# jiwoon-ahn/irn

Measured on AMD Instinct MI355X. Metric: images/sec for CAM+random-walk label gen, VOC12 512^2 (random-walk label generation stage), higher is better.
Workload: dtype f32

## Files before the change

### irn_amd/csrc/affinity.hip

```cpp
#include "path_unroll.hpp"

namespace irn {

namespace {

__device__ __forceinline__ float pow_beta(float a, float beta, int beta_int) {
    double b = (double)a;
    if (beta_int > 0) {
        double r = 1.0;
        int e = beta_int;
        while (e) {
            if (e & 1) r *= b;
            b *= b;
            e >>= 1;
        }
        return (float)r;
    }
    return (float)pow(b, (double)beta);
}

template <bool POW>
__global__ __launch_bounds__(256) void affinity_kernel(const AffJob *__restrict__ jobs,
                                                       const int *__restrict__ dir_start8,
                                                       const int *__restrict__ cell_off8, int n_dirs,
// ... 24 lines not shown
    const bool valid = sy < J.sh && sx < J.sw;
    const int base = ly * LW + lx + halo;
    float *out = J.out + (long)sy * J.sw + sx;

    const float *tb = tile + base;
    for (int d = 0; d < n_dirs; ++d) {
        const int k0 = dir_start8[d], k1 = dir_start8[d + 1];
        float m0 = -INFINITY, m1 = -INFINITY;
        for (int k = k0; k < k1; k += 8) {
            const int4 oa = *reinterpret_cast<const int4 *>(cell_off8 + k);
            const int4 ob = *reinterpret_cast<const int4 *>(cell_off8 + k + 4);
            const float a0 = tb[oa.x], a1 = tb[oa.y], a2 = tb[oa.z], a3 = tb[oa.w];
            const float b0 = tb[ob.x], b1 = tb[ob.y], b2 = tb[ob.z], b3 = tb[ob.w];
            m0 = max3(max3(m0, a0, a1), a2, a3);
            m1 = max3(max3(m1, b0, b1), b2, b3);
        }
        const float m = max3(m0, m1, m1);
        float a = 1.0f - m;
        if (POW) a = pow_beta(a, beta, beta_int);
        if (valid) out[(long)d * J.plane_stride] = a;
    }
}

template <int R>
__global__ __launch_bounds__(256) void affinity_unrolled_kernel(const AffJob *__restrict__ jobs, int beta_int) {
    constexpr int HALO = R - 1, LW = AFF_TW + 2 * HALO, LH = AFF_TH + HALO, ND = kPaths<R>.n_dirs;
    __shared__ float tile[LH * LW];
    const AffJob J = jobs[blockIdx.y];
    const int tiles_x = (J.sw + AFF_TW - 1) / AFF_TW;
    const int tiles_y = (J.sh + AFF_TH - 1) / AFF_TH;
    if ((int)blockIdx.x >= tiles_x * tiles_y) return;
    const int ty0 = ((int)blockIdx.x / tiles_x) * AFF_TH;
    const int tx0 = ((int)blockIdx.x % tiles_x) * AFF_TW;
    for (int i = threadIdx.x; i < LH * LW; i += 256) {
        const int ly = i / LW, lx = i - ly * LW;
        const int gy = J.oy + ty0 + ly;
        const int gx = J.ox + tx0 + lx - HALO;
        float v = 1.0f;
        if (gy < J.gh && gx >= 0 && gx < J.gw) v = J.edge[(long)gy * J.gw + gx];
        tile[i] = v;
    }
    __syncthreads();
    const int ly = threadIdx.x / AFF_TW, lx = threadIdx.x % AFF_TW;
    const int sy = ty0 + ly, sx = tx0 + lx;
    const bool valid = sy < J.sh && sx < J.sw;
    const float *tb = tile + ly * LW + lx;
    float *out = J.out + (long)sy * J.sw + sx;
    static_for<ND>([&](auto id) __attribute__((always_inline)) {
        constexpr int d = decltype(id)::value;
        double b = (double)(1.0f - path_max<R, d>(tb)), r = 1.0;
        for (int e = beta_int; e; e >>= 1) {
            if (e & 1) r *= b;
            b *= b;
        }
        if (valid) *out = (float)r;
        out += J.plane_stride;
    });
}

__global__ __launch_bounds__(256) void affinity_backward_kernel(const AffJob *__restrict__ jobs,
                                                                const float *const *__restrict__ grad_aff,
                                                                float *const *__restrict__ grad_edge,
                                                                const int *__restrict__ dir_start,
                                                                const int *__restrict__ cell_dy,
                                                                const int *__restrict__ cell_dx, int n_dirs, int radius) {
    extern __shared__ float tile[];
    const AffJob J = jobs[blockIdx.y];
    const int tiles_x = (J.sw + AFF_TW - 1) / AFF_TW;
    const int tiles_y = (J.sh + AFF_TH - 1) / AFF_TH;
    if ((int)blockIdx.x >= tiles_x * tiles_y) return;
    const int halo = radius - 1;
    const int LW = AFF_TW + 2 * halo;
    const int LH = AFF_TH + halo;
    float *gtile = tile + LH * LW;
    const int ty0 = ((int)blockIdx.x / tiles_x) * AFF_TH;
    const int tx0 = ((int)blockIdx.x % tiles_x) * AFF_TW;
    for (int i = threadIdx.x; i < LH * LW; i += 256) {
        const int ly = i / LW, lx = i - ly * LW;
        const int gy = J.oy + ty0 + ly;
// ... 19 lines not shown
                const float v = tile[base + off];
                if (v > m) {
                    m = v;
                    arg = off;
                }
            }
            atomicAdd(&gtile[base + arg], -ga[(long)d * J.plane_stride]);
        }
    }
    __syncthreads();
    float *ge = grad_edge[blockIdx.y];
    for (int i = threadIdx.x; i < LH * LW; i += 256) {
        const float g = gtile[i];
        if (g == 0.f) continue;
        const int py = i / LW, px = i - py * LW;
        const int gy = J.oy + ty0 + py;
        const int gx = J.ox + tx0 + px - halo;
        if (gy < J.gh && gx >= 0 && gx < J.gw) unsafeAtomicAdd(ge + (long)gy * J.gw + gx, g);
    }
}

}

int launch_affinity(const AffJob *jobs_dev, int n_jobs, int max_sh, int max_sw, const DeviceTable &tab,
                    bool with_pow, float beta, hipStream_t stream) {
    const int tiles = cdiv(max_sh, AFF_TH) * cdiv(max_sw, AFF_TW);
    const int halo = tab.radius - 1;
    const size_t lds = sizeof(float) * (AFF_TH + halo) * (AFF_TW + 2 * halo);
    dim3 grid(tiles, n_jobs);
    int beta_int = 0;
    if (with_pow && beta == (float)(int)beta && beta >= 1.0f && beta <= 64.0f) beta_int = (int)beta;
    if (with_pow && beta_int > 0 && tab.order == 1 && tab.radius == 10)
        hipLaunchKernelGGL(affinity_unrolled_kernel<10>, grid, dim3(256), 0, stream, jobs_dev, beta_int);
    else if (with_pow && beta_int > 0 && tab.order == 1 && tab.radius == 5)
        hipLaunchKernelGGL(affinity_unrolled_kernel<5>, grid, dim3(256), 0, stream, jobs_dev, beta_int);
    else if (with_pow)
        hipLaunchKernelGGL(affinity_kernel<true>, grid, dim3(256), lds, stream, jobs_dev, tab.dir_start8,
                           tab.cell_off8, tab.n_dirs, tab.radius, beta, beta_int);
    else
        hipLaunchKernelGGL(affinity_kernel<false>, grid, dim3(256), lds, stream, jobs_dev, tab.dir_start8,
                           tab.cell_off8, tab.n_dirs, tab.radius, beta, beta_int);
    IRN_LAUNCH_CHECK("affinity_kernel");
    return IRN_OK;
}

}

using namespace irn;

extern "C" int irn_version(void) { return 100; }

extern "C" const char *irn_last_error(void) { return last_error_slot().c_str(); }

extern "C" int irn_path_count(int radius, int *n_dirs, int *n_cells) {
    if (radius < 2 || radius > IRN_MAX_RADIUS || !n_dirs || !n_cells)
        return fail(IRN_ERR_ARG, "irn_path_count: radius must be in [2,%d]", IRN_MAX_RADIUS);
    PathTable t = build_path_table(radius, 0);
    *n_dirs = t.n_dirs();
// ... 160 lines not shown
```

### irn_amd/csrc/kernels.hpp

```cpp
#pragma once
#include "common.hpp"

namespace irn {

struct DeviceTable {
    int radius = 0, order = 0, n_dirs = 0, n_cells = 0;
    int *dir_dy = nullptr, *dir_dx = nullptr;
    int *dir_start = nullptr;
    int *cell_dy = nullptr, *cell_dx = nullptr;
    int *cell_off8 = nullptr;
    int *dir_start8 = nullptr;
    int *plane_tab = nullptr;
    PathTable host;
};

int get_device_table(int radius, int order, const DeviceTable **out);

int scratch_upload(const void *host, size_t bytes, void **dev_out, hipStream_t stream);
int scratch_release(hipStream_t stream);

constexpr int kAffTileH = 8, kAffTileW = 32;

struct AffJob {
    const float *edge;
    float *out;
    int gh, gw;
    int oy, ox;
    int sh, sw;
    long plane_stride;
};

int launch_affinity(const AffJob *jobs_dev, int n_jobs, int max_sh, int max_sw, const DeviceTable &tab,
                    bool with_pow, float beta, hipStream_t stream);

}
```

### irn_amd/csrc/label.hip

```cpp
#include "kernels.hpp"

#pragma clang fp contract(off)

namespace irn {

struct LabelJob {
    const float *rw;
    const int64_t *keys;
    uint8_t *labels;
    int32_t *argmax;
    float *rw_up;
    unsigned *max_slot;
    int c, h, w, oh, ow;
};

namespace {

__device__ __forceinline__ unsigned enc_ordered(float f) {
    const unsigned b = __float_as_uint(f);
    return (b & 0x80000000u) ? ~b : (b | 0x80000000u);
}
__device__ __forceinline__ float dec_ordered(unsigned u) {
    return __uint_as_float((u & 0x80000000u) ? (u & 0x7fffffffu) : ~u);
}
// ... 7 lines not shown
    float src = ((float)dst + 0.5f) * 0.25f;
    src = src - 0.5f;
    src = src < 0.f ? 0.f : src;
    Taps t;
    t.i0 = min((int)src, n_in - 1);
    t.i1 = min(t.i0 + 1, n_in - 1);
    t.l1 = src - (float)t.i0;
    t.l0 = 1.0f - t.l1;
    return t;
}

__device__ __forceinline__ float bilerp(const float *__restrict__ plane, int w, const Taps &ty, const Taps &tx) {
    const float v00 = plane[ty.i0 * w + tx.i0], v01 = plane[ty.i0 * w + tx.i1];
    const float v10 = plane[ty.i1 * w + tx.i0], v11 = plane[ty.i1 * w + tx.i1];
    const float p01 = v01 * tx.l1, p11 = v11 * tx.l1;
    const float top = __builtin_fmaf(v00, tx.l0, p01);
    const float bot = __builtin_fmaf(v10, tx.l0, p11);
    const float pb = ty.l1 * bot;
    return __builtin_fmaf(ty.l0, top, pb);
}

__device__ __forceinline__ int cell_lo(int k) { return k == 0 ? 0 : 4 * k + 2; }

template <int PASS>
__global__ __launch_bounds__(256) void upsample_max_kernel(const LabelJob *__restrict__ jobs) {
    const LabelJob J = jobs[blockIdx.y];
    const unsigned plane_px = (unsigned)(J.h * J.w), cells = (unsigned)J.c * plane_px;
    const float lower = PASS == 2 ? dec_ordered(*J.max_slot) : 0.f;
    float m = -INFINITY;
    for (unsigned i = blockIdx.x * 256 + threadIdx.x; i < cells; i += gridDim.x * 256) {
        const int c = (int)(i / plane_px);
        const int r = (int)(i - (unsigned)c * plane_px);
        const int k = (int)((unsigned)r / (unsigned)J.w), l = r - k * J.w;
        const int y0 = cell_lo(k), x0 = cell_lo(l);
        if (y0 >= J.oh || x0 >= J.ow) continue;
        const float *plane = J.rw + (long)c * J.h * J.w;
        if (PASS == 1) {
            m = fmaxf(m, bilerp(plane, J.w, taps_x4(y0, J.h), taps_x4(x0, J.w)));
        } else {
            const int k1 = min(k + 1, J.h - 1), l1 = min(l + 1, J.w - 1);
            const float u = fmaxf(fmaxf(plane[k * J.w + l], plane[k * J.w + l1]), fmaxf(plane[k1 * J.w + l], plane[k1 * J.w + l1]));
            if (u + fabsf(u) * 1e-6f + 1e-37f < lower) continue;
            const int y1 = min(k == J.h - 1 ? 4 * J.h - 1 : 4 * k + 5, J.oh - 1);
            const int x1 = min(l == J.w - 1 ? 4 * J.w - 1 : 4 * l + 5, J.ow - 1);
            for (int oy = y0; oy <= y1; ++oy) {
                const Taps ty = taps_x4(oy, J.h);
                for (int ox = x0; ox <= x1; ++ox) m = fmaxf(m, bilerp(plane, J.w, ty, taps_x4(ox, J.w)));
            }
        }
    }
    for (int s = 32; s > 0; s >>= 1) m = fmaxf(m, __shfl_xor(m, s));
    __shared__ float wmax[4];
    if ((threadIdx.x & 63) == 0) wmax[threadIdx.x >> 6] = m;
    __syncthreads();
    if (threadIdx.x == 0) {
        m = fmaxf(fmaxf(wmax[0], wmax[1]), fmaxf(wmax[2], wmax[3]));
        if (m > -INFINITY) atomicMax(J.max_slot, enc_ordered(m));
    }
}

__device__ __forceinline__ float bilerp_vals(float v00, float v01, float v10, float v11, const Taps &ty, const Taps &tx) {
    const float p01 = v01 * tx.l1, p11 = v11 * tx.l1;
    const float top = __builtin_fmaf(v00, tx.l0, p01);
    const float bot = __builtin_fmaf(v10, tx.l0, p11);
    const float pb = ty.l1 * bot;
    return __builtin_fmaf(ty.l0, top, pb);
}

__global__ __launch_bounds__(256) void label_argmax_kernel(const LabelJob *__restrict__ jobs, float bg) {
    const LabelJob J = jobs[blockIdx.y];
    const unsigned gw = (unsigned)(J.ow + 3) >> 2, groups = gw * (unsigned)J.oh;
    const unsigned npx = (unsigned)J.oh * (unsigned)J.ow;
    const float gmax = dec_ordered(*J.max_slot);
    for (unsigned g = blockIdx.x * 256 + threadIdx.x; g < groups; g += gridDim.x * 256) {
        const int oy = (int)(g / gw), ox = (int)(g - (unsigned)oy * gw) * 4;
        const int nq = min(4, J.ow - ox);
        const Taps ty = taps_x4(oy, J.h);
        Taps tx[4];
#pragma unroll
        for (int q = 0; q < 4; ++q) tx[q] = taps_x4(min(ox + q, J.ow - 1), J.w);
        float best[4] = {bg, bg, bg, bg};
// ... 122 lines not shown
            out_h[i] > 4 * h[i] || out_w[i] > 4 * w[i])
            return fail(IRN_ERR_ARG, "irn_label_epilogue: image %d: bad sizes (c=%d %dx%d -> %dx%d)", i, c[i], h[i],
                        w[i], out_h[i], out_w[i]);
        J.rw = rw_dev[i];
        J.keys = keys_dev ? keys_dev[i] : nullptr;
        J.labels = labels_dev ? labels_dev[i] : nullptr;
        J.argmax = argmax_dev ? argmax_dev[i] : nullptr;
        J.rw_up = rw_up_dev ? rw_up_dev[i] : nullptr;
        if (J.labels && !J.keys)
            return fail(IRN_ERR_ARG, "irn_label_epilogue: image %d: labels requested without keys", i);
        J.max_slot = (unsigned *)scratch_dev + i;
        J.c = c[i]; J.h = h[i]; J.w = w[i]; J.oh = out_h[i]; J.ow = out_w[i];
        max_px = std::max(max_px, (long)out_h[i] * out_w[i]);
        max_cells = std::max(max_cells, (long)c[i] * h[i] * w[i]);
    }
    LabelJob *jobs_dev = nullptr;
    int rc = scratch_upload(jobs.data(), sizeof(LabelJob) * n_images, (void **)&jobs_dev, stream);
    if (rc) return rc;
    IRN_HIP_TRY(hipMemsetAsync(scratch_dev, 0, sizeof(unsigned) * n_images, stream));
    if (max_px >= (1L << 31) || max_cells >= (1L << 31)) return fail(IRN_ERR_ARG, "irn_label_epilogue: image too large (32-bit pixel indices)");
    const long per_image = std::max<long>(1, 4096 / n_images);
    const int bx = (int)std::min<long>((max_px / 4 + 255) / 256 + 1, 512);
    const int bc = (int)std::min<long>((max_cells + 255) / 256, per_image);
    hipLaunchKernelGGL(upsample_max_kernel<1>, dim3(bc, n_images), dim3(256), 0, stream, jobs_dev);
    IRN_LAUNCH_CHECK("upsample_max_kernel<1>");
    hipLaunchKernelGGL(upsample_max_kernel<2>, dim3(bc, n_images), dim3(256), 0, stream, jobs_dev);
    IRN_LAUNCH_CHECK("upsample_max_kernel<2>");
    hipLaunchKernelGGL(label_argmax_kernel, dim3(bx, n_images), dim3(256), 0, stream, jobs_dev, bg_thres);
    IRN_LAUNCH_CHECK("label_argmax_kernel");
    return scratch_release(stream);
}

extern "C" int irn_cam_merge(int n_scales, const float *const *src_dev, const int32_t *hs, const int32_t *ws, int n_classes,
                             const int64_t *keys_dev, int n_keys, int out_h, int out_w, float *cam_dev,
                             float *high_res_dev, void *scratch_dev, void *stream_) {
    hipStream_t stream = (hipStream_t)stream_;
    if (n_scales < 1 || n_scales > kMaxScales || !src_dev || !hs || !ws || n_classes < 1 || !keys_dev || n_keys < 1 ||
        out_h < 1 || out_w < 1 || !cam_dev || !high_res_dev || !scratch_dev)
        return fail(IRN_ERR_ARG, "irn_cam_merge: bad argument (1..%d scales, >= 1 key)", kMaxScales);
    MergeArgs A;
    for (int s = 0; s < n_scales; ++s) {
        if (!src_dev[s] || hs[s] < 1 || ws[s] < 1) return fail(IRN_ERR_ARG, "irn_cam_merge: scale %d: bad input", s);
        A.src[s] = src_dev[s];
        A.hs[s] = hs[s];
        A.ws[s] = ws[s];
    }
    A.n_scales = n_scales;
    A.n_cls = n_classes;
    A.k = n_keys;
    A.keys = keys_dev;
// ... 18 lines not shown
```

### irn_amd/csrc/path_unroll.hpp

```cpp
#pragma once
#include <utility>

#include "kernels.hpp"

namespace irn {

constexpr int AFF_TH = kAffTileH;
constexpr int AFF_TW = kAffTileW;

__device__ __forceinline__ float max3(float a, float b, float c) {
    float r;
    asm("v_max3_f32 %0, %1, %2, %3" : "=v"(r) : "v"(a), "v"(b), "v"(c));
    return r;
}

template <int R>
struct Paths {
    static constexpr int kMaxDirs = 2 * R * R, kMaxCells = 32 * R * R;
    int n_dirs = 0, n_cells = 0;
    signed char dy[kMaxDirs] = {}, dx[kMaxDirs] = {};
    short start[kMaxDirs + 1] = {};
    signed char cy[kMaxCells] = {}, cx[kMaxCells] = {};
    constexpr void add(int y, int x) {
        dy[n_dirs] = (signed char)y;
        dx[n_dirs] = (signed char)x;
        const int lsq = y * y + x * x;
        const int x_lo = x < 0 ? x : 0, x_hi = x < 0 ? 0 : x;
        for (int py = 0; py <= y; ++py)
            for (int px = x_lo; px <= x_hi; ++px) {
                const int cross = y * px - x * py;
                if (cross * cross < lsq) {
                    cy[n_cells] = (signed char)py;
                    cx[n_cells] = (signed char)px;
                    ++n_cells;
                }
            }
        start[++n_dirs] = (short)n_cells;
    }
    constexpr Paths() {
        for (int x = 1; x < R; ++x) add(0, x);
        for (int y = 1; y < R; ++y)
            for (int x = -R + 1; x < R; ++x)
                if (x * x + y * y < R * R) add(y, x);
    }
};
template <int R>
inline constexpr Paths<R> kPaths{};

template <int... Is, typename F>
__device__ __forceinline__ void static_for_impl(std::integer_sequence<int, Is...>, F &&f) {
    (f(std::integral_constant<int, Is>{}), ...);
}
template <int N, typename F>
__device__ __forceinline__ void static_for(F &&f) {
    static_for_impl(std::make_integer_sequence<int, N>{}, f);
}

template <int R, int D>
__device__ __forceinline__ float path_max(const float *tb) {
    constexpr int LW = AFF_TW + 2 * (R - 1), HALO = R - 1;
    constexpr int k0 = kPaths<R>.start[D], n = kPaths<R>.start[D + 1] - k0;
    constexpr auto off = [](int k) constexpr { return kPaths<R>.cy[k] * LW + kPaths<R>.cx[k] + HALO; };
    float m = tb[off(k0)];
    static_for<(n - 1) / 2>([&](auto ik) __attribute__((always_inline)) {
        constexpr int k = k0 + 1 + 2 * decltype(ik)::value;
        m = max3(m, tb[off(k)], tb[off(k + 1)]);
    });
    if constexpr ((n - 1) % 2 == 1) {
        const float v = tb[off(k0 + n - 1)];
        m = max3(m, v, v);
    }
    return m;
}

}
```

### irn_amd/csrc/walk.hip

```cpp
#include <algorithm>
#include <cmath>
#include <mutex>

#include "walk_ctx.hpp"

namespace irn {


namespace {


__global__ __launch_bounds__(256) void zero_pad_kernel(const WalkImg *__restrict__ imgs, int n_dirs) {
    const WalkImg I = imgs[blockIdx.y];
    const int d = blockIdx.x;
    if (d >= n_dirs) return;
    float *plane = I.wts + (long)d * I.plane_stride;
    for (int i = threadIdx.x; i < I.front_pad; i += 256) plane[-1 - i] = 0.f;
    const long n = (long)I.h * I.w;
    const long end = I.plane_stride - I.front_pad;
    for (long i = n + threadIdx.x; i < end; i += 256) plane[i] = 0.f;
}

__global__ __launch_bounds__(256) void degree_kernel(const WalkImg *__restrict__ imgs,
                                                     const int *__restrict__ dir_dy,
                                                     const int *__restrict__ dir_dx, int n_dirs) {
    const WalkImg I = imgs[blockIdx.y];
    const long n = (long)I.h * I.w;
    const long p = (long)blockIdx.x * 256 + threadIdx.x;
    if (p >= n) return;
    const int y = (int)(p / I.w), x = (int)(p - (long)y * I.w);
    double deg = 1.0;
    for (int d = 0; d < n_dirs; ++d) {
        const int dy = dir_dy[d], dx = dir_dx[d];
        const float *plane = I.wts + (long)d * I.plane_stride;
        deg += (double)plane[p];
        const int yy = y - dy, xx = x - dx;
        if (yy >= 0 && xx >= 0 && xx < I.w) deg += (double)plane[p - ((long)dy * I.w + dx)];
    }
    I.inv_deg[p] = 1.0 / deg;
}

__global__ __launch_bounds__(256) void x0_kernel(const WalkImg *__restrict__ imgs, int to_out, int cheb, float c0) {
    const WalkImg I = imgs[blockIdx.y];
// ... 721 lines not shown
        I.out = out_dev[i];
        I.wts = (float *)(ws + ctx->off_wts[i]) + ctx->front_pad[i];
        I.inv_deg = (double *)(ws + ctx->off_deg[i]);
        I.xa = (float *)(ws + ctx->off_xa[i]);
        I.xb = (float *)(ws + ctx->off_xb[i]);
        I.xc = (float *)(ws + ctx->off_xc[i]);
        I.h = ctx->h[i];
        I.w = ctx->w[i];
        I.C = ctx->c[i];
        I.plane_stride = ctx->plane_stride[i];
        I.front_pad = ctx->front_pad[i];
        I.n_dirs = ctx->tab->n_dirs;
        AffJob &J = jobs[i];
        J.edge = I.edge;
        J.out = I.wts;
        J.gh = I.h; J.gw = I.w; J.oy = 0; J.ox = 0; J.sh = I.h; J.sw = I.w;
        J.plane_stride = I.plane_stride;
    }
    IRN_HIP_TRY(hipMemcpyAsync(ctx->imgs_dev, imgs, sizeof(WalkImg) * n, hipMemcpyHostToDevice, stream));
    IRN_HIP_TRY(hipMemcpyAsync(ctx->jobs_dev, jobs, sizeof(AffJob) * n, hipMemcpyHostToDevice, stream));
    IRN_HIP_TRY(hipEventRecord(ctx->stage_ev[slot], stream));

    const DeviceTable &tab = *ctx->tab;
    hipLaunchKernelGGL(zero_pad_kernel, dim3(tab.n_dirs, n), dim3(256), 0, stream, ctx->imgs_dev, tab.n_dirs);
    IRN_LAUNCH_CHECK("zero_pad_kernel");
    int rc = launch_affinity(ctx->jobs_dev, n, ctx->max_h, ctx->max_w, tab, true, beta, stream);
    if (rc) return rc;
    const bool resident = ctx->variant == 2 && ctx->res_ok && n_sweeps > 0;
    ctx->deg_stale = resident;
    ctx->last_stream = stream;
    ctx->last_n_sweeps = n_sweeps;
    ctx->last_resident = resident;
    ctx->last_valid = true;
    hipEvent_t ev0 = nullptr, ev1 = nullptr;
    if (ctx->timing && resident) {
        rc = timing_events(ctx, &ev0, &ev1);
        if (rc) return rc;
        IRN_HIP_TRY(hipEventRecord(ev0, stream));
    }
    if (resident) {
        rc = resident_run(ctx, n_sweeps, stream);
        if (rc) return rc;
        if (ctx->timing) {
            IRN_HIP_TRY(hipEventRecord(ev1, stream));
            ctx->ev_used += 2;
            ctx->pending_launches += ctx->sched_steps;
        }
    } else {
        rc = streaming_run(ctx, n_sweeps, stream, ctx->timing != 0);
        if (rc) return rc;
    }
    if (!ctx->run_done_ev) IRN_HIP_TRY(hipEventCreateWithFlags(&ctx->run_done_ev, hipEventDisableTiming));
    IRN_HIP_TRY(hipEventRecord(ctx->run_done_ev, stream));
    return IRN_OK;
}

extern "C" int irn_walk_check(irn_walk_ctx *ctx) {
    if (!ctx) return fail(IRN_ERR_ARG, "null ctx");
    if (!ctx->res_err_host) return IRN_OK;
    if (ctx->res_err_host[0] != 0) {
        const unsigned img = ctx->res_err_host[1], t = ctx->res_err_host[2], wg = ctx->res_err_host[3];
        ctx->res_err_host[0] = 0;
        return fail(IRN_ERR_STATE, "resident walk timed out: workgroup %u waiting for state of sweep %u of image %u "
                                   "(a neighbouring tile never published it)", wg, t, img);
// ... 79 lines not shown
```

### irn_amd/csrc/walk_ctx.hpp

```cpp
#pragma once
#include <utility>
#include <vector>

#include "kernels.hpp"

namespace irn {

struct WalkImg {
    const float *edge;
    const float *cam;
    const int *inst;
    float *out;
    float *wts;
    double *inv_deg;
    float *xa, *xb;
    float *xc;
    int h, w, C, k_inst;
    long plane_stride;
    int front_pad, n_dirs;
};

#define IRN_GLOBAL __attribute__((address_space(1)))

template <int R>
__host__ __device__ constexpr bool in_set(int dy, int dx) {
    return dy == 0 ? (dx >= 1 && dx < R) : (dy < R && dx > -R && dx < R && dx * dx + dy * dy < R * R);
}

template <int R>
__host__ __device__ constexpr int plane_of(int dy, int dx) {
    int n = 0;
    for (int y = 0; y < R; ++y)
        for (int x = -R + 1; x < R; ++x) {
            if (y == dy && x == dx) return n;
            if (in_set<R>(y, x)) ++n;
        }
    return -1;
}

template <int... Is, typename F>
__device__ __forceinline__ void static_for_impl(std::integer_sequence<int, Is...>, F &&f) {
    (f(std::integral_constant<int, Is>{}), ...);
}
template <int N, typename F>
__device__ __forceinline__ void static_for(F &&f) {
    static_for_impl(std::make_integer_sequence<int, N>{}, f);
}

}

struct irn_walk_ctx {
    using DeviceTable = irn::DeviceTable;
    using WalkImg = irn::WalkImg;
    using AffJob = irn::AffJob;
    int radius = 0;
    const DeviceTable *tab = nullptr;
    int variant = 1;
    hipStream_t side[3] = {nullptr, nullptr, nullptr};
    hipEvent_t ev_fork = nullptr, ev_join[3] = {nullptr, nullptr, nullptr};
    int n = 0;
    std::vector<int> h, w, c;
    std::vector<size_t> off_wts, off_deg, off_xa, off_xb, off_xc;
    std::vector<long> plane_stride;
    std::vector<int> front_pad;
    size_t ws_bytes = 0;
    int max_h = 0, max_w = 0, max_n = 0;
    bool all_blocked_ok = false;
    WalkImg *imgs_dev = nullptr;
    AffJob *jobs_dev = nullptr;
// ... 31 lines not shown
    bool res_coop_refused = false;
    int res_inject_timeout = 0;
    hipStream_t last_stream = nullptr;
    hipEvent_t run_done_ev = nullptr;
    bool last_valid = false, last_resident = false;
    int last_n_sweeps = 0;
    int fallback_runs = 0;
    int accel = 1;
    int accel_tol_exp = 7;
    int sched_n = -1, sched_accel = -1, sched_tol = -1;
    int sched_steps = 0;
    bool sched_cheb = false;
    float *coef_dev = nullptr;
    std::vector<double> sched_coef;
    std::vector<float> sched_coef_f;
    int coef_cap = 0;
};

namespace irn {
bool resident_supported(const irn_walk_ctx *ctx);
int resident_configure(irn_walk_ctx *ctx);
bool resident_plan_rounds(int radius, int n, const int *h, const int *w, const int *c, int n_wg, int placement,
                          std::vector<int> &jobs, int *n_rounds);
int resident_run(irn_walk_ctx *ctx, int n_sweeps, hipStream_t stream);
int walk_schedule(irn_walk_ctx *ctx, int n_sweeps, hipStream_t stream);
int chebyshev_power_series(int n, double tol, std::vector<double> *coef, bool *cheb);
int streaming_run(irn_walk_ctx *ctx, int n_sweeps, hipStream_t stream, bool timed);
void resident_destroy(irn_walk_ctx *ctx);
}
```

### irn_amd/csrc/walk_resident.hip

```cpp
#include <algorithm>
#include <mutex>

#include "walk_ctx.hpp"

namespace irn {
namespace {

typedef unsigned long long u64;
typedef const double IRN_GLOBAL *gcd_t;
typedef float IRN_GLOBAL *gf_t;
typedef float f4a __attribute__((ext_vector_type(4)));

constexpr int kSlabH = 8, kSlabW = 32;
constexpr int kWaves = 8;
constexpr int kPsLdsBytes = 96 * 1024;

template <int R>
struct RCfg;
template <>
struct RCfg<10> {
    static constexpr int Q = 8, SL_Y = 1, SL_X = 1;
};
template <>
struct RCfg<5> {
    static constexpr int Q = 2, SL_Y = 2, SL_X = 2;
};

template <int R>
struct Disc {
    int n = 0;
    signed char dy[4 * R * R] = {}, dx[4 * R * R] = {};
// ... 189 lines not shown
typedef unsigned u4v __attribute__((ext_vector_type(4)));
constexpr int kSc1 = 16;
__device__ __forceinline__ u2v ld_granule(__amdgpu_buffer_rsrc_t rsrc, int voff, int soff) {
    return __builtin_bit_cast(u2v, __builtin_amdgcn_raw_buffer_load_b64(rsrc, voff, soff, kSc1));
}
template <int AUX = kSc1>
__device__ __forceinline__ void st_granule(__amdgpu_buffer_rsrc_t rsrc, int voff, int soff, unsigned tag, float v) {
    u2v g;
    g.x = __float_as_uint(v);
    g.y = tag;
    __builtin_amdgcn_raw_buffer_store_b64(g, rsrc, voff, soff, AUX);
}

template <int AUX = kSc1>
__device__ __forceinline__ void st_granule2(__amdgpu_buffer_rsrc_t rsrc, int voff, int soff, unsigned tag, float v0, float v1) {
    u4v g;
    g.x = __float_as_uint(v0);
    g.y = tag;
    g.z = __float_as_uint(v1);
    g.w = tag;
    __builtin_amdgcn_raw_buffer_store_b128(g, rsrc, voff, soff, AUX);
}

typedef float f2a __attribute__((ext_vector_type(2)));
__global__ __launch_bounds__(256) void x0_granule_kernel(const WalkImg *__restrict__ imgs, int cheb, float c0) {
    const WalkImg I = imgs[blockIdx.y];
    const long n = (long)I.h * I.w;
    const long p = (long)blockIdx.x * 256 + threadIdx.x;
    if (p >= n) return;
    const float one_minus = 1.0f - I.edge[p];
    const int k = I.inst ? I.k_inst : 1;
    const int id = I.inst ? I.inst[p] : 0;
    u64 *xa = (u64 *)I.xa, *xb = (u64 *)I.xb;
    for (int c = 0; c < I.C; ++c) {
        const int cls = c / k, kk = c - cls * k;
        float v = I.cam[(long)cls * n + p];
        if (I.inst) v = v * (id == kk ? 1.0f : 0.0f);
        xa[(long)c * n + p] = ((u64)1 << 32) | (u64)__float_as_uint(v * one_minus);
        xb[(long)c * n + p] = 0;
        if (cheb) ((f2a *)I.xc)[(long)c * n + p] = f2a{0.f, c0 * (v * one_minus)};
    }
}

__global__ __launch_bounds__(64) void xcc_probe_kernel(unsigned char *__restrict__ out) {
    if (threadIdx.x == 0) out[blockIdx.x] = (unsigned char)((unsigned)__builtin_amdgcn_s_getreg((31 << 11) | 20) & 7u);
}

template <int R, bool PROF>
__global__ __launch_bounds__(512) __attribute__((amdgpu_waves_per_eu(2, 2))) void resident_kernel(
    const WalkImg *__restrict__ imgs, const int4 *__restrict__ jobs, int n_rounds, int t_first, int t_count,
    int t_total, unsigned *err, long long timeout_ticks, long long *prof, int poll_delay, unsigned long long *votes,
    const float *__restrict__ coef, int cheb) {
    using G = Geom<R>;
    constexpr int H = G::H, HP = G::HP, LH = G::LH, LW = G::LW, LWU = G::LWU, RG = G::RG, Q = G::Q, NK = G::NK;
    extern __shared__ __attribute__((aligned(16))) char smem[];
    float *xs = reinterpret_cast<float *>(smem);
    double *part = reinterpret_cast<double *>(smem + G::XS_BYTES);
    double *invd = reinterpret_cast<double *>(smem + G::XS_BYTES + G::PART_BYTES);
    int *abort_flag = reinterpret_cast<int *>(smem + G::XS_BYTES + G::PART_BYTES + G::INVD_BYTES);
    f2a *psl = reinterpret_cast<f2a *>(smem + G::PS_OFF);

    const int tid = threadIdx.x;
    const int lane = tid & 63;
    const int wv = __builtin_amdgcn_readfirstlane(tid >> 6);
// ... 660 lines not shown
    }
    const WalkImg *imgs = ctx->imgs_dev;
    const int4 *jobs = ctx->res_jobs_dev;
    int n_rounds = ctx->res_rounds;
    unsigned *err = ctx->res_err_dev;
    long long *prof = ctx->res_prof_dev;
    int delays = ctx->res_poll_delay | (ctx->res_poll_delay_plain << 16);
    const float *coef = ctx->coef_dev;
    int cheb = ctx->sched_cheb ? 1 : 0;
    if (ctx->res_cooperative && !ctx->res_coop_refused) {
        void *args[] = {&imgs, &jobs, &n_rounds, &t_first, &t_count, &t_total, &err, &ticks, &prof, &delays, &votes, &coef, &cheb};
        const hipError_t e = hipLaunchCooperativeKernel((const void *)resident_kernel<R, PROF>, dim3(ctx->res_nwg), dim3(512),
                                                        args, G::LDS_BYTES, stream);
        if (e == hipSuccess) return IRN_OK;
        (void)hipGetLastError();
        ctx->res_coop_refused = true;
    }
    hipLaunchKernelGGL((resident_kernel<R, PROF>), dim3(ctx->res_nwg), dim3(512), G::LDS_BYTES, stream, imgs, jobs, n_rounds,
                       t_first, t_count, t_total, err, ticks, prof, delays, votes, coef, cheb);
    IRN_LAUNCH_CHECK("resident_kernel");
    return IRN_OK;
}

static int resident_enqueue(irn_walk_ctx *ctx, hipStream_t stream) {
    const int n = ctx->n;
    const int n_sweeps = ctx->sched_steps;
    IRN_HIP_TRY(hipMemsetAsync(ctx->res_err_dev, 0, 4 * sizeof(unsigned), stream));
    hipLaunchKernelGGL(x0_granule_kernel, dim3(cdiv(ctx->max_n, 256), n), dim3(256), 0, stream, ctx->imgs_dev,
                       ctx->sched_cheb ? 1 : 0, ctx->sched_cheb ? (float)ctx->sched_coef[0] : 0.f);
    IRN_LAUNCH_CHECK("x0_granule_kernel");
    const int step = ctx->res_sweeps_per_launch > 0 ? ctx->res_sweeps_per_launch : n_sweeps;
    for (int t = 0; t < n_sweeps; t += step) {
        const int cnt = std::min(step, n_sweeps - t);
        int rc;
        if (ctx->res_prof_dev)
            rc = ctx->radius == 10 ? launch_resident<10, true>(ctx, t, cnt, n_sweeps, stream)
                                   : launch_resident<5, true>(ctx, t, cnt, n_sweeps, stream);
        else
            rc = ctx->radius == 10 ? launch_resident<10, false>(ctx, t, cnt, n_sweeps, stream)
                                   : launch_resident<5, false>(ctx, t, cnt, n_sweeps, stream);
        if (rc) return rc;
    }
    IRN_HIP_TRY(hipMemcpyAsync(ctx->res_err_host, ctx->res_err_dev, 4 * sizeof(unsigned), hipMemcpyDeviceToHost, stream));
    return IRN_OK;
}

static int g_poll_delay[64] = {};

static int resident_probe_poll_delay(irn_walk_ctx *ctx, hipStream_t stream) {
    int dev = 0;
    IRN_HIP_TRY(hipGetDevice(&dev));
    if (dev < 0 || dev >= 64 || ctx->radius != 10 || !ctx->res_poll_auto) return IRN_OK;
    std::lock_guard<std::mutex> lk(g_tune_mu);
    if (g_poll_delay[dev]) {
        ctx->res_poll_delay = g_poll_delay[dev];
        return IRN_OK;
    }
    if (ctx->res_prof_dev || ctx->res_sweeps_per_launch > 0 || ctx->res_inject_timeout || ctx->res_rounds < 4 ||
        ctx->sched_steps < 32)
        return IRN_OK;
    int single = 0;
    for (int i = 0; i < ctx->n; ++i) single += ctx->c[i] == 1 ? 1 : 0;
    if (3 * single < ctx->n) return IRN_OK;
    hipEvent_t e0, e1;
    IRN_HIP_TRY(hipEventCreate(&e0));
    IRN_HIP_TRY(hipEventCreate(&e1));
    constexpr int NC = 4;
    const int cand[NC] = {10, 8, 12, 14};
    float best_ms[NC] = {1e30f, 1e30f, 1e30f, 1e30f};
    int rc = IRN_OK;
    for (int rep = 0; rep < 2 && !rc; ++rep)
        for (int k = 0; k < NC && !rc; ++k) {
            ctx->res_poll_delay = cand[k];
            (void)hipEventRecord(e0, stream);
            rc = resident_enqueue(ctx, stream);
            (void)hipEventRecord(e1, stream);
            if (rc) break;
            if (hipEventSynchronize(e1) != hipSuccess) { rc = fail(IRN_ERR_HIP, "poll-delay probe: synchronisation failed"); break; }
            float ms = 0.f;
            (void)hipEventElapsedTime(&ms, e0, e1);
            if (ctx->res_err_host[0] != 0) ms = 1e30f;
            best_ms[k] = std::min(best_ms[k], ms);
        }
    (void)hipEventDestroy(e0);
    (void)hipEventDestroy(e1);
    int pick = 0;
    for (int k = 1; k < NC; ++k)
        if (best_ms[k] < 0.993f * best_ms[0] && best_ms[k] < best_ms[pick]) pick = k;
    ctx->res_poll_delay = cand[pick];
    ctx->res_poll_probe_ms[0] = best_ms[1];
    ctx->res_poll_probe_ms[1] = best_ms[0];
    ctx->res_poll_probe_ms[2] = best_ms[2];
    ctx->res_poll_probe_ms[3] = best_ms[3];
    if (!rc && best_ms[0] < 1e29f) g_poll_delay[dev] = cand[pick];
    return rc;
}

int resident_run(irn_walk_ctx *ctx, int n_sweeps, hipStream_t stream) {
    {
        const int rc_s = walk_schedule(ctx, n_sweeps, stream);
        if (rc_s) return rc_s;
    }
    {
        const int rc_p = resident_probe_poll_delay(ctx, stream);
        if (rc_p) return rc_p;
    }
    return resident_enqueue(ctx, stream);
}

}
```

Measured before the change: 19280.

## Fuse walk setup into affinity kernel, nest path maxima, single-launch upsample max

The unrolled affinity kernel gains extra blocks that zero the wts plane padding and initialise the x0 granules, which removes the separate zero_pad and x0_granule launches on the resident path. Each direction's path maximum now starts from a parent direction whose cell set is a subset (a compile-time forest), which cuts the LDS reads per pixel considerably. Beta is specialised at compile time for beta=10. The two-pass upsample_max kernels are merged into one kernel that takes its pruning bound from a per-block atomicMax between the passes. That gives a weaker bound than the old global one and may prune less.

```diff
diff --git a/irn_amd/csrc/affinity.hip b/irn_amd/csrc/affinity.hip
--- a/irn_amd/csrc/affinity.hip
+++ b/irn_amd/csrc/affinity.hip
@@ -1,4 +1,5 @@
 #include "path_unroll.hpp"
+#include "walk_setup.hpp"
 
 namespace irn {
 
@@ -70,10 +71,18 @@
     }
 }
 
-template <int R>
-__global__ __launch_bounds__(256) void affinity_unrolled_kernel(const AffJob *__restrict__ jobs, int beta_int) {
+template <int R, int BETA>
+__global__ __launch_bounds__(256) void affinity_unrolled_kernel(const AffJob *__restrict__ jobs, int beta_int, int tiles,
+                                                                AffSetup setup) {
     constexpr int HALO = R - 1, LW = AFF_TW + 2 * HALO, LH = AFF_TH + HALO, ND = kPaths<R>.n_dirs;
     __shared__ float tile[LH * LW];
+    if ((int)blockIdx.x >= tiles) {
+        const WalkImg I = setup.imgs[blockIdx.y];
+        const int b = (int)blockIdx.x - tiles;
+        if (b < ND) zero_pad_plane(I, b);
+        else x0_granules(I, (long)(b - ND) * 256 + threadIdx.x, setup.cheb, setup.c0);
+        return;
+    }
     const AffJob J = jobs[blockIdx.y];
     const int tiles_x = (J.sw + AFF_TW - 1) / AFF_TW;
     const int tiles_y = (J.sh + AFF_TH - 1) / AFF_TH;
@@ -91,18 +100,28 @@
     __syncthreads();
     const int ly = threadIdx.x / AFF_TW, lx = threadIdx.x % AFF_TW;
     const int sy = ty0 + ly, sx = tx0 + lx;
-    const bool valid = sy < J.sh && sx < J.sw;
+    if (sy >= J.sh || sx >= J.sw) return;
     const float *tb = tile + ly * LW + lx;
-    float *out = J.out + (long)sy * J.sw + sx;
-    static_for<ND>([&](auto id) __attribute__((always_inline)) {
-        constexpr int d = decltype(id)::value;
-        double b = (double)(1.0f - path_max<R, d>(tb)), r = 1.0;
-        for (int e = beta_int; e; e >>= 1) {
-            if (e & 1) r *= b;
-            b *= b;
+    typedef __attribute__((address_space(1))) float gfloat;
+    const unsigned pix = (unsigned)sy * (unsigned)J.sw + (unsigned)sx;
+    float chain[kForest<R>.max_depth + 1];
+    static_for<ND>([&](auto ii) __attribute__((always_inline)) {
+        constexpr int i = decltype(ii)::value, d = kForest<R>.order[i];
+        double b = (double)(1.0f - nested_path_max<R, i>(tb, chain)), r = 1.0;
+        if constexpr (BETA > 0) {
+            static_for<32 - __builtin_clz(BETA)>([&](auto ie) __attribute__((always_inline)) {
+                constexpr int e = BETA >> decltype(ie)::value;
+                if constexpr (e & 1) r *= b;
+                if constexpr (e > 1) b *= b;
+            });
+        } else {
+            for (int e = beta_int; e; e >>= 1) {
+                if (e & 1) r *= b;
+                b *= b;
+            }
         }
-        if (valid) *out = (float)r;
-        out += J.plane_stride;
+        ((gfloat *)(J.out + d * J.plane_stride))[pix] = (float)r;
+        if constexpr (i % 4 == 3) __builtin_amdgcn_sched_barrier(0);
     });
 }
 
@@ -168,18 +187,32 @@
 
 }
 
+static int affinity_beta_int(bool with_pow, float beta) {
+    return with_pow && beta == (float)(int)beta && beta >= 1.0f && beta <= 64.0f ? (int)beta : 0;
+}
+
+bool affinity_has_setup_roles(const DeviceTable &tab, float beta) {
+    return affinity_beta_int(true, beta) > 0 && tab.order == 1 && (tab.radius == 5 || tab.radius == 10);
+}
+
 int launch_affinity(const AffJob *jobs_dev, int n_jobs, int max_sh, int max_sw, const DeviceTable &tab,
-                    bool with_pow, float beta, hipStream_t stream) {
+                    bool with_pow, float beta, hipStream_t stream, const AffSetup *setup) {
     const int tiles = cdiv(max_sh, AFF_TH) * cdiv(max_sw, AFF_TW);
     const int halo = tab.radius - 1;
     const size_t lds = sizeof(float) * (AFF_TH + halo) * (AFF_TW + 2 * halo);
-    dim3 grid(tiles, n_jobs);
-    int beta_int = 0;
-    if (with_pow && beta == (float)(int)beta && beta >= 1.0f && beta <= 64.0f) beta_int = (int)beta;
-    if (with_pow && beta_int > 0 && tab.order == 1 && tab.radius == 10)
-        hipLaunchKernelGGL(affinity_unrolled_kernel<10>, grid, dim3(256), 0, stream, jobs_dev, beta_int);
-    else if (with_pow && beta_int > 0 && tab.order == 1 && tab.radius == 5)
-        hipLaunchKernelGGL(affinity_unrolled_kernel<5>, grid, dim3(256), 0, stream, jobs_dev, beta_int);
+    const int beta_int = affinity_beta_int(with_pow, beta);
+    const bool unrolled = beta_int > 0 && tab.order == 1 && (tab.radius == 5 || tab.radius == 10);
+    if (setup && !unrolled) return fail(IRN_ERR_STATE, "launch_affinity: this kernel has no set-up roles");
+    const AffSetup su = setup ? *setup : AffSetup{nullptr, 0, 0, 0.f};
+    dim3 grid(tiles + (setup ? tab.n_dirs + su.x0_blocks : 0), n_jobs);
+    if (unrolled && beta_int == 10 && tab.radius == 10)
+        hipLaunchKernelGGL((affinity_unrolled_kernel<10, 10>), grid, dim3(256), 0, stream, jobs_dev, beta_int, tiles, su);
+    else if (unrolled && beta_int == 10)
+        hipLaunchKernelGGL((affinity_unrolled_kernel<5, 10>), grid, dim3(256), 0, stream, jobs_dev, beta_int, tiles, su);
+    else if (unrolled && tab.radius == 10)
+        hipLaunchKernelGGL((affinity_unrolled_kernel<10, 0>), grid, dim3(256), 0, stream, jobs_dev, beta_int, tiles, su);
+    else if (unrolled)
+        hipLaunchKernelGGL((affinity_unrolled_kernel<5, 0>), grid, dim3(256), 0, stream, jobs_dev, beta_int, tiles, su);
     else if (with_pow)
         hipLaunchKernelGGL(affinity_kernel<true>, grid, dim3(256), lds, stream, jobs_dev, tab.dir_start8,
                            tab.cell_off8, tab.n_dirs, tab.radius, beta, beta_int);
diff --git a/irn_amd/csrc/kernels.hpp b/irn_amd/csrc/kernels.hpp
--- a/irn_amd/csrc/kernels.hpp
+++ b/irn_amd/csrc/kernels.hpp
@@ -30,7 +30,9 @@
     long plane_stride;
 };
 
+struct AffSetup;
+bool affinity_has_setup_roles(const DeviceTable &tab, float beta);
 int launch_affinity(const AffJob *jobs_dev, int n_jobs, int max_sh, int max_sw, const DeviceTable &tab,
-                    bool with_pow, float beta, hipStream_t stream);
+                    bool with_pow, float beta, hipStream_t stream, const AffSetup *setup = nullptr);
 
 }
diff --git a/irn_amd/csrc/label.hip b/irn_amd/csrc/label.hip
--- a/irn_amd/csrc/label.hip
+++ b/irn_amd/csrc/label.hip
@@ -53,11 +53,19 @@
 
 __device__ __forceinline__ int cell_lo(int k) { return k == 0 ? 0 : 4 * k + 2; }
 
-template <int PASS>
+__device__ __forceinline__ float block_max(float m, float *slot) {
+    for (int s = 32; s > 0; s >>= 1) m = fmaxf(m, __shfl_xor(m, s));
+    __syncthreads();
+    if ((threadIdx.x & 63) == 0) slot[threadIdx.x >> 6] = m;
+    __syncthreads();
+    return fmaxf(fmaxf(slot[0], slot[1]), fmaxf(slot[2], slot[3]));
+}
+
 __global__ __launch_bounds__(256) void upsample_max_kernel(const LabelJob *__restrict__ jobs) {
     const LabelJob J = jobs[blockIdx.y];
     const unsigned plane_px = (unsigned)(J.h * J.w), cells = (unsigned)J.c * plane_px;
-    const float lower = PASS == 2 ? dec_ordered(*J.max_slot) : 0.f;
+    __shared__ float wmax[4];
+    __shared__ float lower_s;
     float m = -INFINITY;
     for (unsigned i = blockIdx.x * 256 + threadIdx.x; i < cells; i += gridDim.x * 256) {
         const int c = (int)(i / plane_px);
@@ -65,29 +73,37 @@
         const int k = (int)((unsigned)r / (unsigned)J.w), l = r - k * J.w;
         const int y0 = cell_lo(k), x0 = cell_lo(l);
         if (y0 >= J.oh || x0 >= J.ow) continue;
+        m = fmaxf(m, bilerp(J.rw + (long)c * J.h * J.w, J.w, taps_x4(y0, J.h), taps_x4(x0, J.w)));
+    }
+    m = block_max(m, wmax);
+    if (threadIdx.x == 0) {
+        unsigned seen = 0;
+        if (m > -INFINITY) seen = max(atomicMax(J.max_slot, enc_ordered(m)), enc_ordered(m));
+        lower_s = seen ? dec_ordered(seen) : -INFINITY;
+    }
+    __syncthreads();
+    const float lower = lower_s;
+    if (!(m > -INFINITY)) return;
+    m = -INFINITY;
+    for (unsigned i = blockIdx.x * 256 + threadIdx.x; i < cells; i += gridDim.x * 256) {
+        const int c = (int)(i / plane_px);
+        const int r = (int)(i - (unsigned)c * plane_px);
+        const int k = (int)((unsigned)r / (unsigned)J.w), l = r - k * J.w;
+        const int y0 = cell_lo(k), x0 = cell_lo(l);
+        if (y0 >= J.oh || x0 >= J.ow) continue;
         const float *plane = J.rw + (long)c * J.h * J.w;
-        if (PASS == 1) {
-            m = fmaxf(m, bilerp(plane, J.w, taps_x4(y0, J.h), taps_x4(x0, J.w)));
-        } else {
-            const int k1 = min(k + 1, J.h - 1), l1 = min(l + 1, J.w - 1);
-            const float u = fmaxf(fmaxf(plane[k * J.w + l], plane[k * J.w + l1]), fmaxf(plane[k1 * J.w + l], plane[k1 * J.w + l1]));
-            if (u + fabsf(u) * 1e-6f + 1e-37f < lower) continue;
-            const int y1 = min(k == J.h - 1 ? 4 * J.h - 1 : 4 * k + 5, J.oh - 1);
-            const int x1 = min(l == J.w - 1 ? 4 * J.w - 1 : 4 * l + 5, J.ow - 1);
-            for (int oy = y0; oy <= y1; ++oy) {
-                const Taps ty = taps_x4(oy, J.h);
-                for (int ox = x0; ox <= x1; ++ox) m = fmaxf(m, bilerp(plane, J.w, ty, taps_x4(ox, J.w)));
-            }
-        }
-    }
-    for (int s = 32; s > 0; s >>= 1) m = fmaxf(m, __shfl_xor(m, s));
-    __shared__ float wmax[4];
-    if ((threadIdx.x & 63) == 0) wmax[threadIdx.x >> 6] = m;
-    __syncthreads();
-    if (threadIdx.x == 0) {
-        m = fmaxf(fmaxf(wmax[0], wmax[1]), fmaxf(wmax[2], wmax[3]));
-        if (m > -INFINITY) atomicMax(J.max_slot, enc_ordered(m));
-    }
+        const int k1 = min(k + 1, J.h - 1), l1 = min(l + 1, J.w - 1);
+        const float u = fmaxf(fmaxf(plane[k * J.w + l], plane[k * J.w + l1]), fmaxf(plane[k1 * J.w + l], plane[k1 * J.w + l1]));
+        if (u + fabsf(u) * 1e-6f + 1e-37f < lower) continue;
+        const int y1 = min(k == J.h - 1 ? 4 * J.h - 1 : 4 * k + 5, J.oh - 1);
+        const int x1 = min(l == J.w - 1 ? 4 * J.w - 1 : 4 * l + 5, J.ow - 1);
+        for (int oy = y0; oy <= y1; ++oy) {
+            const Taps ty = taps_x4(oy, J.h);
+            for (int ox = x0; ox <= x1; ++ox) m = fmaxf(m, bilerp(plane, J.w, ty, taps_x4(ox, J.w)));
+        }
+    }
+    m = block_max(m, wmax);
+    if (threadIdx.x == 0 && m > -INFINITY) atomicMax(J.max_slot, enc_ordered(m));
 }
 
 __device__ __forceinline__ float bilerp_vals(float v00, float v01, float v10, float v11, const Taps &ty, const Taps &tx) {
@@ -256,10 +272,8 @@
     const long per_image = std::max<long>(1, 4096 / n_images);
     const int bx = (int)std::min<long>((max_px / 4 + 255) / 256 + 1, 512);
     const int bc = (int)std::min<long>((max_cells + 255) / 256, per_image);
-    hipLaunchKernelGGL(upsample_max_kernel<1>, dim3(bc, n_images), dim3(256), 0, stream, jobs_dev);
-    IRN_LAUNCH_CHECK("upsample_max_kernel<1>");
-    hipLaunchKernelGGL(upsample_max_kernel<2>, dim3(bc, n_images), dim3(256), 0, stream, jobs_dev);
-    IRN_LAUNCH_CHECK("upsample_max_kernel<2>");
+    hipLaunchKernelGGL(upsample_max_kernel, dim3(bc, n_images), dim3(256), 0, stream, jobs_dev);
+    IRN_LAUNCH_CHECK("upsample_max_kernel");
     hipLaunchKernelGGL(label_argmax_kernel, dim3(bx, n_images), dim3(256), 0, stream, jobs_dev, bg_thres);
     IRN_LAUNCH_CHECK("label_argmax_kernel");
     return scratch_release(stream);
diff --git a/irn_amd/csrc/path_unroll.hpp b/irn_amd/csrc/path_unroll.hpp
--- a/irn_amd/csrc/path_unroll.hpp
+++ b/irn_amd/csrc/path_unroll.hpp
@@ -1,7 +1,6 @@
 #pragma once
-#include <utility>
-
 #include "kernels.hpp"
+#include "static_for.hpp"
 
 namespace irn {
 
@@ -47,15 +46,6 @@
 template <int R>
 inline constexpr Paths<R> kPaths{};
 
-template <int... Is, typename F>
-__device__ __forceinline__ void static_for_impl(std::integer_sequence<int, Is...>, F &&f) {
-    (f(std::integral_constant<int, Is>{}), ...);
-}
-template <int N, typename F>
-__device__ __forceinline__ void static_for(F &&f) {
-    static_for_impl(std::make_integer_sequence<int, N>{}, f);
-}
-
 template <int R, int D>
 __device__ __forceinline__ float path_max(const float *tb) {
     constexpr int LW = AFF_TW + 2 * (R - 1), HALO = R - 1;
@@ -73,4 +63,97 @@
     return m;
 }
 
+template <int R>
+struct Forest {
+    static constexpr int kMaxDirs = Paths<R>::kMaxDirs, kMaxCells = Paths<R>::kMaxCells;
+    static constexpr int kRowBits = 2 * R - 1, kWords = (R * kRowBits + 63) / 64;
+    struct Mask {
+        unsigned long long w[kWords] = {};
+        int count = 0;
+        constexpr void set(int y, int x) {
+            const int b = y * kRowBits + x + R - 1;
+            w[b / 64] |= 1ull << (b % 64);
+            ++count;
+        }
+        constexpr bool has(int y, int x) const {
+            const int b = y * kRowBits + x + R - 1;
+            return (w[b / 64] >> (b % 64)) & 1ull;
+        }
+        constexpr bool within(const Mask &o) const {
+            for (int i = 0; i < kWords; ++i)
+                if (w[i] & ~o.w[i]) return false;
+            return true;
+        }
+    };
+    int n_dirs = 0, n_cells = 0, max_depth = 0, operands = 0;
+    short parent[kMaxDirs] = {}, order[kMaxDirs] = {}, depth[kMaxDirs] = {};
+    short start[kMaxDirs + 1] = {};
+    signed char cy[kMaxCells] = {}, cx[kMaxCells] = {};
+    bool exact = true;
+    Mask mask[kMaxDirs] = {};
+
+    constexpr void visit(const Paths<R> &P, int d, int dep) {
+        const int i = n_dirs++;
+        order[i] = (short)d;
+        depth[i] = (short)dep;
+        if (dep > max_depth) max_depth = dep;
+        Mask got = dep ? mask[parent[d]] : Mask{};
+        for (int k = P.start[d]; k < P.start[d + 1]; ++k)
+            if (!dep || !mask[parent[d]].has(P.cy[k], P.cx[k])) {
+                if (got.has(P.cy[k], P.cx[k])) exact = false;
+                got.set(P.cy[k], P.cx[k]);
+                cy[n_cells] = P.cy[k];
+                cx[n_cells] = P.cx[k];
+                ++n_cells;
+            }
+        start[i + 1] = (short)n_cells;
+        operands += start[i + 1] - start[i] + (dep ? 1 : 0);
+        if (got.count != mask[d].count || !got.within(mask[d]) || !mask[d].within(got)) exact = false;
+        for (int c = 0; c < P.n_dirs; ++c)
+            if (parent[c] == d) visit(P, c, dep + 1);
+    }
+    constexpr Forest() {
+        const Paths<R> &P = kPaths<R>;
+        for (int d = 0; d < P.n_dirs; ++d)
+            for (int k = P.start[d]; k < P.start[d + 1]; ++k) mask[d].set(P.cy[k], P.cx[k]);
+        for (int d = 0; d < P.n_dirs; ++d) {
+            int best = -1;
+            for (int e = 0; e < P.n_dirs; ++e) {
+                if (e == d || mask[e].count >= mask[d].count || (best >= 0 && mask[e].count <= mask[best].count)) continue;
+                if (mask[e].within(mask[d])) best = e;
+            }
+            parent[d] = (short)best;
+        }
+        for (int d = 0; d < P.n_dirs; ++d)
+            if (parent[d] < 0) visit(P, d, 0);
+    }
+};
+template <int R>
+inline constexpr Forest<R> kForest{};
+
+static_assert(kForest<5>.n_dirs == kPaths<5>.n_dirs && kForest<10>.n_dirs == kPaths<10>.n_dirs, "every direction is emitted once");
+static_assert(kForest<5>.exact && kForest<10>.exact, "path(parent(d)) + extra(d) must be path(d)");
+static_assert(kForest<5>.operands == 110 && kPaths<5>.n_cells == 242, "operands per pixel at radius 5");
+static_assert(kForest<10>.operands == 798 && kPaths<10>.n_cells == 2134, "operands per pixel at radius 10");
+
+template <int R, int I>
+__device__ __forceinline__ float nested_path_max(const float *tb, float (&m)[kForest<R>.max_depth + 1]) {
+    constexpr int LW = AFF_TW + 2 * (R - 1), HALO = R - 1;
+    constexpr int dep = kForest<R>.depth[I], k0 = kForest<R>.start[I] + (dep ? 0 : 1), n = kForest<R>.start[I + 1] - k0;
+    constexpr auto off = [](int k) constexpr { return kForest<R>.cy[k] * LW + kForest<R>.cx[k] + HALO; };
+    float v;
+    if constexpr (dep > 0) v = m[dep - 1];
+    else v = tb[off(k0 - 1)];
+    static_for<n / 2>([&](auto ik) __attribute__((always_inline)) {
+        constexpr int k = k0 + 2 * decltype(ik)::value;
+        v = max3(v, tb[off(k)], tb[off(k + 1)]);
+    });
+    if constexpr (n % 2 == 1) {
+        const float u = tb[off(k0 + n - 1)];
+        v = max3(v, u, u);
+    }
+    m[dep] = v;
+    return v;
 }
+
+}
diff --git a/irn_amd/csrc/static_for.hpp b/irn_amd/csrc/static_for.hpp
--- /dev/null
+++ b/irn_amd/csrc/static_for.hpp
@@ -0,0 +1,15 @@
+#pragma once
+#include <utility>
+
+namespace irn {
+
+template <int... Is, typename F>
+__device__ __forceinline__ void static_for_impl(std::integer_sequence<int, Is...>, F &&f) {
+    (f(std::integral_constant<int, Is>{}), ...);
+}
+template <int N, typename F>
+__device__ __forceinline__ void static_for(F &&f) {
+    static_for_impl(std::make_integer_sequence<int, N>{}, f);
+}
+
+}
diff --git a/irn_amd/csrc/walk.hip b/irn_amd/csrc/walk.hip
--- a/irn_amd/csrc/walk.hip
+++ b/irn_amd/csrc/walk.hip
@@ -12,13 +12,7 @@
 
 __global__ __launch_bounds__(256) void zero_pad_kernel(const WalkImg *__restrict__ imgs, int n_dirs) {
     const WalkImg I = imgs[blockIdx.y];
-    const int d = blockIdx.x;
-    if (d >= n_dirs) return;
-    float *plane = I.wts + (long)d * I.plane_stride;
-    for (int i = threadIdx.x; i < I.front_pad; i += 256) plane[-1 - i] = 0.f;
-    const long n = (long)I.h * I.w;
-    const long end = I.plane_stride - I.front_pad;
-    for (long i = n + threadIdx.x; i < end; i += 256) plane[i] = 0.f;
+    if ((int)blockIdx.x < n_dirs) zero_pad_plane(I, blockIdx.x);
 }
 
 __global__ __launch_bounds__(256) void degree_kernel(const WalkImg *__restrict__ imgs,
@@ -786,11 +780,21 @@
     IRN_HIP_TRY(hipEventRecord(ctx->stage_ev[slot], stream));
 
     const DeviceTable &tab = *ctx->tab;
-    hipLaunchKernelGGL(zero_pad_kernel, dim3(tab.n_dirs, n), dim3(256), 0, stream, ctx->imgs_dev, tab.n_dirs);
-    IRN_LAUNCH_CHECK("zero_pad_kernel");
-    int rc = launch_affinity(ctx->jobs_dev, n, ctx->max_h, ctx->max_w, tab, true, beta, stream);
+    const bool resident = ctx->variant == 2 && ctx->res_ok && n_sweeps > 0;
+    const bool fused_setup = resident && affinity_has_setup_roles(tab, beta);
+    int rc = IRN_OK;
+    if (fused_setup) {
+        rc = walk_schedule(ctx, n_sweeps, stream);
+        if (rc) return rc;
+        const AffSetup su{ctx->imgs_dev, cdiv(ctx->max_n, 256), ctx->sched_cheb ? 1 : 0,
+                          ctx->sched_cheb ? (float)ctx->sched_coef[0] : 0.f};
+        rc = launch_affinity(ctx->jobs_dev, n, ctx->max_h, ctx->max_w, tab, true, beta, stream, &su);
+    } else {
+        hipLaunchKernelGGL(zero_pad_kernel, dim3(tab.n_dirs, n), dim3(256), 0, stream, ctx->imgs_dev, tab.n_dirs);
+        IRN_LAUNCH_CHECK("zero_pad_kernel");
+        rc = launch_affinity(ctx->jobs_dev, n, ctx->max_h, ctx->max_w, tab, true, beta, stream);
+    }
     if (rc) return rc;
-    const bool resident = ctx->variant == 2 && ctx->res_ok && n_sweeps > 0;
     ctx->deg_stale = resident;
     ctx->last_stream = stream;
     ctx->last_n_sweeps = n_sweeps;
@@ -803,7 +807,7 @@
         IRN_HIP_TRY(hipEventRecord(ev0, stream));
     }
     if (resident) {
-        rc = resident_run(ctx, n_sweeps, stream);
+        rc = resident_run(ctx, n_sweeps, stream, fused_setup);
         if (rc) return rc;
         if (ctx->timing) {
             IRN_HIP_TRY(hipEventRecord(ev1, stream));
diff --git a/irn_amd/csrc/walk_ctx.hpp b/irn_amd/csrc/walk_ctx.hpp
--- a/irn_amd/csrc/walk_ctx.hpp
+++ b/irn_amd/csrc/walk_ctx.hpp
@@ -3,22 +3,10 @@
 #include <vector>
 
 #include "kernels.hpp"
+#include "static_for.hpp"
+#include "walk_setup.hpp"
 
 namespace irn {
-
-struct WalkImg {
-    const float *edge;
-    const float *cam;
-    const int *inst;
-    float *out;
-    float *wts;
-    double *inv_deg;
-    float *xa, *xb;
-    float *xc;
-    int h, w, C, k_inst;
-    long plane_stride;
-    int front_pad, n_dirs;
-};
 
 #define IRN_GLOBAL __attribute__((address_space(1)))
 
@@ -36,15 +24,6 @@
             if (in_set<R>(y, x)) ++n;
         }
     return -1;
-}
-
-template <int... Is, typename F>
-__device__ __forceinline__ void static_for_impl(std::integer_sequence<int, Is...>, F &&f) {
-    (f(std::integral_constant<int, Is>{}), ...);
-}
-template <int N, typename F>
-__device__ __forceinline__ void static_for(F &&f) {
-    static_for_impl(std::make_integer_sequence<int, N>{}, f);
 }
 
 }
@@ -122,7 +101,7 @@
 int resident_configure(irn_walk_ctx *ctx);
 bool resident_plan_rounds(int radius, int n, const int *h, const int *w, const int *c, int n_wg, int placement,
                           std::vector<int> &jobs, int *n_rounds);
-int resident_run(irn_walk_ctx *ctx, int n_sweeps, hipStream_t stream);
+int resident_run(irn_walk_ctx *ctx, int n_sweeps, hipStream_t stream, bool x0_done);
 int walk_schedule(irn_walk_ctx *ctx, int n_sweeps, hipStream_t stream);
 int chebyshev_power_series(int n, double tol, std::vector<double> *coef, bool *cheb);
 int streaming_run(irn_walk_ctx *ctx, int n_sweeps, hipStream_t stream, bool timed);
diff --git a/irn_amd/csrc/walk_resident.hip b/irn_amd/csrc/walk_resident.hip
--- a/irn_amd/csrc/walk_resident.hip
+++ b/irn_amd/csrc/walk_resident.hip
@@ -6,7 +6,6 @@
 namespace irn {
 namespace {
 
-typedef unsigned long long u64;
 typedef const double IRN_GLOBAL *gcd_t;
 typedef float IRN_GLOBAL *gf_t;
 typedef float f4a __attribute__((ext_vector_type(4)));
@@ -242,24 +241,9 @@
     __builtin_amdgcn_raw_buffer_store_b128(g, rsrc, voff, soff, AUX);
 }
 
-typedef float f2a __attribute__((ext_vector_type(2)));
 __global__ __launch_bounds__(256) void x0_granule_kernel(const WalkImg *__restrict__ imgs, int cheb, float c0) {
     const WalkImg I = imgs[blockIdx.y];
-    const long n = (long)I.h * I.w;
-    const long p = (long)blockIdx.x * 256 + threadIdx.x;
-    if (p >= n) return;
-    const float one_minus = 1.0f - I.edge[p];
-    const int k = I.inst ? I.k_inst : 1;
-    const int id = I.inst ? I.inst[p] : 0;
-    u64 *xa = (u64 *)I.xa, *xb = (u64 *)I.xb;
-    for (int c = 0; c < I.C; ++c) {
-        const int cls = c / k, kk = c - cls * k;
-        float v = I.cam[(long)cls * n + p];
-        if (I.inst) v = v * (id == kk ? 1.0f : 0.0f);
-        xa[(long)c * n + p] = ((u64)1 << 32) | (u64)__float_as_uint(v * one_minus);
-        xb[(long)c * n + p] = 0;
-        if (cheb) ((f2a *)I.xc)[(long)c * n + p] = f2a{0.f, c0 * (v * one_minus)};
-    }
+    x0_granules(I, (long)blockIdx.x * 256 + threadIdx.x, cheb, c0);
 }
 
 __global__ __launch_bounds__(64) void xcc_probe_kernel(unsigned char *__restrict__ out) {
@@ -966,13 +950,15 @@
     return IRN_OK;
 }
 
-static int resident_enqueue(irn_walk_ctx *ctx, hipStream_t stream) {
+static int resident_enqueue(irn_walk_ctx *ctx, hipStream_t stream, bool x0_done) {
     const int n = ctx->n;
     const int n_sweeps = ctx->sched_steps;
     IRN_HIP_TRY(hipMemsetAsync(ctx->res_err_dev, 0, 4 * sizeof(unsigned), stream));
-    hipLaunchKernelGGL(x0_granule_kernel, dim3(cdiv(ctx->max_n, 256), n), dim3(256), 0, stream, ctx->imgs_dev,
-                       ctx->sched_cheb ? 1 : 0, ctx->sched_cheb ? (float)ctx->sched_coef[0] : 0.f);
-    IRN_LAUNCH_CHECK("x0_granule_kernel");
+    if (!x0_done) {
+        hipLaunchKernelGGL(x0_granule_kernel, dim3(cdiv(ctx->max_n, 256), n), dim3(256), 0, stream, ctx->imgs_dev,
+                           ctx->sched_cheb ? 1 : 0, ctx->sched_cheb ? (float)ctx->sched_coef[0] : 0.f);
+        IRN_LAUNCH_CHECK("x0_granule_kernel");
+    }
     const int step = ctx->res_sweeps_per_launch > 0 ? ctx->res_sweeps_per_launch : n_sweeps;
     for (int t = 0; t < n_sweeps; t += step) {
         const int cnt = std::min(step, n_sweeps - t);
@@ -991,7 +977,7 @@
 
 static int g_poll_delay[64] = {};
 
-static int resident_probe_poll_delay(irn_walk_ctx *ctx, hipStream_t stream) {
+static int resident_probe_poll_delay(irn_walk_ctx *ctx, hipStream_t stream, bool *x0_done) {
     int dev = 0;
     IRN_HIP_TRY(hipGetDevice(&dev));
     if (dev < 0 || dev >= 64 || ctx->radius != 10 || !ctx->res_poll_auto) return IRN_OK;
@@ -1017,7 +1003,8 @@
         for (int k = 0; k < NC && !rc; ++k) {
             ctx->res_poll_delay = cand[k];
             (void)hipEventRecord(e0, stream);
-            rc = resident_enqueue(ctx, stream);
+            rc = resident_enqueue(ctx, stream, *x0_done);
+            *x0_done = false;
             (void)hipEventRecord(e1, stream);
             if (rc) break;
             if (hipEventSynchronize(e1) != hipSuccess) { rc = fail(IRN_ERR_HIP, "poll-delay probe: synchronisation failed"); break; }
@@ -1040,16 +1027,16 @@
     return rc;
 }
 
-int resident_run(irn_walk_ctx *ctx, int n_sweeps, hipStream_t stream) {
+int resident_run(irn_walk_ctx *ctx, int n_sweeps, hipStream_t stream, bool x0_done) {
     {
         const int rc_s = walk_schedule(ctx, n_sweeps, stream);
         if (rc_s) return rc_s;
     }
     {
-        const int rc_p = resident_probe_poll_delay(ctx, stream);
+        const int rc_p = resident_probe_poll_delay(ctx, stream, &x0_done);
         if (rc_p) return rc_p;
     }
-    return resident_enqueue(ctx, stream);
-}
-
-}
+    return resident_enqueue(ctx, stream, x0_done);
+}
+
+}
diff --git a/irn_amd/csrc/walk_setup.hpp b/irn_amd/csrc/walk_setup.hpp
--- /dev/null
+++ b/irn_amd/csrc/walk_setup.hpp
@@ -0,0 +1,55 @@
+#pragma once
+#include "kernels.hpp"
+
+namespace irn {
+
+struct WalkImg {
+    const float *edge;
+    const float *cam;
+    const int *inst;
+    float *out;
+    float *wts;
+    double *inv_deg;
+    float *xa, *xb;
+    float *xc;
+    int h, w, C, k_inst;
+    long plane_stride;
+    int front_pad, n_dirs;
+};
+
+
+__device__ __forceinline__ void zero_pad_plane(const WalkImg &I, int d) {
+    float *plane = I.wts + (long)d * I.plane_stride;
+    for (int i = threadIdx.x; i < I.front_pad; i += 256) plane[-1 - i] = 0.f;
+    const long n = (long)I.h * I.w;
+    const long end = I.plane_stride - I.front_pad;
+    for (long i = n + threadIdx.x; i < end; i += 256) plane[i] = 0.f;
+}
+
+typedef unsigned long long u64;
+typedef float f2a __attribute__((ext_vector_type(2)));
+__device__ __forceinline__ void x0_granules(const WalkImg &I, long p, int cheb, float c0) {
+    const long n = (long)I.h * I.w;
+    if (p >= n) return;
+    const float one_minus = 1.0f - I.edge[p];
+    const int k = I.inst ? I.k_inst : 1;
+    const int id = I.inst ? I.inst[p] : 0;
+    u64 *xa = (u64 *)I.xa, *xb = (u64 *)I.xb;
+    for (int c = 0; c < I.C; ++c) {
+        const int cls = c / k, kk = c - cls * k;
+        float v = I.cam[(long)cls * n + p];
+        if (I.inst) v = v * (id == kk ? 1.0f : 0.0f);
+        xa[(long)c * n + p] = ((u64)1 << 32) | (u64)__float_as_uint(v * one_minus);
+        xb[(long)c * n + p] = 0;
+        if (cheb) ((f2a *)I.xc)[(long)c * n + p] = f2a{0.f, c0 * (v * one_minus)};
+    }
+}
+
+struct AffSetup {
+    const WalkImg *imgs;
+    int x0_blocks;
+    int cheb;
+    float c0;
+};
+
+}
```

Measured after the change: 19790, median of 6. 2.6% higher.
